# sydney-machine-learning/parallel-tempering-neural-net

Measured on AMD Instinct MI355X. Metric: MCMC samples/sec (all replicas) + swap-accept rate; Sunspot 64-replica FNN, higher is better.
Workload: dtype f32

## Files before the change

### parallel-tempering-neural-net_amd/csrc/ptnn.hip

```cpp
#include "ptnn_shapes.hpp"
namespace ptnn {
#include "ptnn_dev_swap.hpp"
}
#include "ptnn_host.hpp"

#include <algorithm>
#include <atomic>
#include <cmath>
#include <cstdarg>
#include <cstdio>
#include <cstdlib>
#include <cstring>
#include <memory>
#include <unordered_map>
#include <mutex>
#include <string>
#include <thread>
#include <vector>
#include <sched.h>

using namespace ptnn;

thread_local std::string ptnn::g_err;

// ... 152 lines not shown
void ladder_adapt_release(ptnn_handle* h) {
    for (void* p : {(void*)h->d_lad_hist, (void*)h->d_lad_s, (void*)h->d_lad_acc})
        if (p) (void)hipFree(p);
    h->d_lad_hist = nullptr; h->d_lad_s = nullptr; h->d_lad_acc = nullptr;
    h->have_adapt = false; h->adapt = ptnn_ladder_adapt_spec{};
    h->lad_T0.clear(); h->lad_s0.clear();
}

}

int ptnn::ladder_adapt_alloc(ptnn_handle* h, const ptnn_ladder_adapt_spec& spec) {
    ladder_adapt_release(h);
    const size_t R = h->cfg.n_replicas_global;
    HIP_TRY(hipMalloc(&h->d_lad_hist, (size_t)(spec.rounds + 1) * R * sizeof(float)));
    HIP_TRY(hipMalloc(&h->d_lad_s, 2 * (R - 1) * sizeof(double)));
    HIP_TRY(hipMalloc(&h->d_lad_acc, (size_t)h->max_rounds * (R - 1) * sizeof(float)));
    h->adapt = spec; h->have_adapt = true;
    return 0;
}

namespace {

int ladder_adapt_reset(ptnn_handle* h) {
    const size_t R = h->cfg.n_replicas_global;
    HIP_TRY(hipMemsetAsync(h->d_lad_hist, 0xff, (size_t)(h->adapt.rounds + 1) * R * sizeof(float), h->stream));
    HIP_TRY(hipMemsetAsync(h->d_lad_acc, 0xff, (size_t)h->max_rounds * (R - 1) * sizeof(float), h->stream));
    HIP_TRY(hipMemcpyAsync(h->d_lad_hist, h->lad_T0.data(), R * sizeof(float), hipMemcpyHostToDevice, h->stream));
    HIP_TRY(hipMemcpyAsync(h->d_temps_global, h->lad_T0.data(), R * sizeof(float), hipMemcpyHostToDevice, h->stream));
    HIP_TRY(hipMemcpyAsync(h->d_lad_s, h->lad_s0.data(), (R - 1) * sizeof(double), hipMemcpyHostToDevice, h->stream));
    HIP_TRY(hipStreamSynchronize(h->stream));
    return 0;
}

int launch_segment(ptnn_handle* h, int begin, int end, bool swap_inside = false, bool round_follows = false) {
    if (end <= begin) return 0;
    HIP_TRY(hipSetDevice(h->cfg.device_id));
    SegParams p = h->seg_params();
    if (round_follows && h->comm.kind == COMM_RCCL) { p.seg_progress = h->h_progress + 1; p.seg_ordinal = h->rounds_done + 1; }
    PersistParams pp{};
    pp.end = end; pp.swap_inside = swap_inside ? 1 : 0; pp.task = h->cfg.task; pp.si = h->cfg.swap_interval;
    pp.round0 = h->rounds_done; pp.flip0 = h->flip; pp.lflip0 = h->lflip;
    const int grid = h->plan.grid(h->cfg.n_replicas_local);
    pp.nblocks = grid; pp.barrier = h->d_barrier;
    for (int b = 0; b < 2; ++b) {
        pp.state[b] = h->d_state[b]; pp.gd[b] = h->d_gd_w[b]; pp.gd_valid[b] = h->d_gd_valid[b];
        pp.label[b] = h->d_label[b]; pp.slot_of[b] = h->d_slot_of[b];
    }
    fill_swap_params(h, false, pp.sp);
    if (swap_inside) {
        if (grid > h->barrier_slots) {
            if (h->d_barrier) HIP_TRY(hipFree(h->d_barrier));
            h->d_barrier = nullptr;
            HIP_TRY(hipMalloc(&h->d_barrier, (size_t)grid * sizeof(unsigned)));
            h->barrier_slots = grid;
            pp.barrier = h->d_barrier;
        }
        HIP_TRY(hipMemsetAsync(h->d_barrier, 0, (size_t)grid * sizeof(unsigned), h->stream));
    }
    const bool timed = h->timing_stride > 0 && (h->launch_count++ % h->timing_stride) == 0;
    std::pair<hipEvent_t, hipEvent_t>* ev = nullptr;
    if (timed) {
        if (h->timing_used == h->timing.size()) {
            if (h->timing.size() >= 4096) {
                if (int rc = wait_stream(h)) return rc;
                collect_timing(h);
            } else {
                hipEvent_t a, b;
                HIP_TRY(hipEventCreate(&a));
                HIP_TRY(hipEventCreate(&b));
                h->timing.emplace_back(a, b);
            }
        }
        ev = &h->timing[h->timing_used++];
        HIP_TRY(hipEventRecord(ev->first, h->stream));
    }
    hipLaunchKernelGGL(plan_function(h->shape, h->plan), dim3(grid), dim3(h->plan.threads), h->plan.seg_lds, h->stream, p, pp, begin);
    h->epoch_base += (unsigned)(end - begin) + 1u + (swap_inside ? (unsigned)((end - begin) / h->cfg.swap_interval + 2) : 0u);
    HIP_TRY(hipGetLastError());
    if (ev) HIP_TRY(hipEventRecord(ev->second, h->stream));
    return 0;
}

int launch_swap(ptnn_handle* h, bool phantom, int mode, bool want_src) {
    HIP_TRY(hipSetDevice(h->cfg.device_id));
    SwapParams sp{};
    fill_swap_params(h, phantom, sp);
    sp.src_out = want_src ? h->d_src : nullptr;
    sp.progress = (mode >= 0 && (mode & 2)) ? h->h_progress : nullptr;
    if (mode == -1) {
        hipLaunchKernelGGL(xchg_pack_kernel, dim3(sp.Rl), dim3(64), 0, h->stream, sp);
// ... 263 lines not shown
        if (explicit_tree && want) break;
    }
    if (explicit_tree)
        return fail(-3, "tree schedule: %d replicas x %d work-groups of %d threads cannot all be resident on %d CUs (or need more than "
                        "160 KiB of LDS)", Rl, want ? want : 3, threads, h.num_cus);
    return 0;
}

int plan_persistent(const ptnn_handle& h, LaunchPlan& plan) {
    const ptnn_config& c = h.cfg;
    const char* e = std::getenv("PTNN_PERSISTENT");
    if ((e && e[0] == '0') || c.shared_device) return 0;
    const bool forced = e && e[0] == '1';
    const int R = c.n_replicas_global;
    const bool whole = c.swap_rule == 0 && !c.label_swap && plan.xswap > 0 && c.n_replicas_local == R;
    const bool tree_inside = plan.kind == SEG_TREE && whole && R <= TREE_PERSIST_MAX_R;
    const bool packm_inside = plan.kind == SEG_PACKM && whole && (size_t)(3 * R + 1) <= (size_t)pack_slots(plan.pk_nred) * pack_slot_floats(h.PS);
    const bool own_rounds = tree_inside || packm_inside;
    if (plan.grid(1) > 1 && !own_rounds && !forced) return 0;
    if (c.swap_interval < 8 && !own_rounds && !forced) return 0;
    if (plan.kind == SEG_SPEC || (plan.kind == SEG_TREE && !tree_inside) || (plan.kind == SEG_PACKM && !packm_inside)) return 0;
    if (plan.kind == SEG_PACK && !(h.shape->loops & 2)) return 0;
    if (plan.kind == SEG_COOP && !(h.shape->loops & 1)) return 0;
    const size_t swap_lds = (size_t)(3 * R + 1) * sizeof(float);
    if (swap_lds > plan.seg_lds) {
        if (swap_lds > LDS_CEILING) return 0;
        plan.seg_lds = swap_lds;
    }
    const void* fn = reinterpret_cast<const void*>(plan_function(h.shape, plan));
    if (int rc = raise_lds_limit(fn, plan.seg_lds)) return rc;
    int per_cu = 0;
    HIP_TRY(hipOccupancyMaxActiveBlocksPerMultiprocessor(&per_cu, fn, plan.threads, plan.seg_lds));
    plan.persistent = (long long)plan.grid(c.n_replicas_local) <= (long long)per_cu * h.num_cus;
    return 0;
}

int plan_launch(const ptnn_handle& h, int Nall, int Npad, LaunchPlan& plan) {
    const ptnn_config& c = h.cfg;
    plan = LaunchPlan{};
    if (c.n_hidden > WAVE) {
        if (int rc = plan_wide(h, plan)) return rc;
    } else {
        plan.model_lds = lds_floats(Nall, h.IPY, h.PS, c.n_hidden, h.FWS) * sizeof(float);
        if (plan.model_lds > LDS_MAX)
            return fail(-3, "replica working set needs %zu B of LDS (> 160 KiB): data %d rows x %d floats, P = %d", plan.model_lds, Nall,
                        h.IPY, h.P);
        int sched = c.schedule;
        if (sched == PTNN_SCHED_AUTO) sched = (c.task == PTNN_TASK_REG || c.use_langevin) ? PTNN_SCHED_SPECULATIVE : PTNN_SCHED_COOPERATIVE;
        if (sched != PTNN_SCHED_COOPERATIVE && sched != PTNN_SCHED_SPECULATIVE && sched != PTNN_SCHED_PACKED && sched != PTNN_SCHED_TREE)
            return fail(-1, "unknown schedule %d", sched);
        if (sched == PTNN_SCHED_TREE && (c.task != PTNN_TASK_CLS || c.use_langevin))
            return fail(-3, "the prefetching tree schedule is built for random-walk classification runs");
        plan.pk_nred = (c.n_hidden <= 8) ? 3 : 4;
        if (int rc = plan_packed(h, Nall, sched, plan)) return rc;
        if (plan.kind != SEG_COOP) sched = PTNN_SCHED_PACKED;
        const int nw = c.waves_per_replica;
        if (nw != 0 && nw != 1 && nw != 2 && nw != 4 && nw != 8) return fail(-1, "waves_per_replica must be 0 (auto), 1, 2, 4 or 8");
        int pow2 = 1;
        while (pow2 < (Nall + 63) / 64) pow2 <<= 1;
        plan.model_threads = std::min(pow2, 8) * 64;
        if (sched == PTNN_SCHED_SPECULATIVE) {
            if (int rc = plan_speculative(h, Nall, plan)) return rc;
            if (plan.kind == SEG_COOP) sched = PTNN_SCHED_COOPERATIVE;
        }
        if (sched == PTNN_SCHED_COOPERATIVE) plan_cooperative(h, Nall, Npad, plan);
        const bool auto_tree = sched == PTNN_SCHED_COOPERATIVE && c.schedule == PTNN_SCHED_AUTO && c.task == PTNN_TASK_CLS &&
// ... 185 lines not shown
    int ndev = 0;
    HIP_TRY(hipGetDeviceCount(&ndev));
    if (cfg->device_id < 0 || cfg->device_id >= ndev) return fail(-2, "device %d not present (%d devices)", cfg->device_id, ndev);
    HIP_TRY(hipSetDevice(cfg->device_id));
    hipDeviceProp_t prop;
    HIP_TRY(hipGetDeviceProperties(&prop, cfg->device_id));
    if (std::strncmp(prop.gcnArchName, "gfx950", 6) != 0)
        return fail(-2, "device %d is %s; libptnn is built for gfx950 only", cfg->device_id, prop.gcnArchName);

    if (cfg->trace_capacity < 0 || (cfg->trace_capacity > 0 && cfg->trace_capacity < 2))
        return fail(-1, "trace_capacity must be 0 (= n_samples) or >= 2");
    ptnn_handle* h = new ptnn_handle();
    if (int rc = create_buffers(h, cfg, sh, prop)) {
        const std::string why = g_err;
        ptnn_destroy(h);
        g_err = why;
        return rc;
    }
    *out = h;
    return 0;
}

int ptnn_destroy(ptnn_handle* h) {
    if (!h) return 0;
    (void)hipSetDevice(h->cfg.device_id);
    if (h->stream && !h->comm.failed) (void)wait_stream(h);
    h->comm.release();
    if (h->comm.failed && h->stream) {
        const double t0 = comm_clock();
        while (hipStreamQuery(h->stream) == hipErrorNotReady && comm_clock() - t0 < 5.0) std::this_thread::sleep_for(std::chrono::milliseconds(1));
        if (hipStreamQuery(h->stream) == hipErrorNotReady) return fail(-7, "the stream of a failed communicator did not drain: handle leaked");
    }
    void* ptrs[] = {h->d_data, h->d_state[0], h->d_state[1], h->d_rec_w, h->d_gd_w[0], h->d_gd_w[1], h->d_gd_valid[0], h->d_gd_valid[1], h->d_st_f, h->d_st_i, h->d_temps,
                    h->d_L_handoff, h->d_L_final, h->d_L_raw, h->d_prior_post, h->d_temps_global, h->d_pos_w, h->d_scal, h->d_src, h->d_label[0], h->d_label[1], h->d_slot_of[0], h->d_slot_of[1], h->d_src_log, h->d_counters, h->d_error, h->d_xslots, h->d_xw, h->d_xverdict, h->d_xswap, h->d_stamps, h->d_wide_scratch, h->d_xt, h->d_xs, h->d_barrier};
    for (void* p : ptrs)
        if (p) (void)hipFree(p);
    if (h->h_src) (void)hipHostFree(h->h_src);
    if (h->h_progress) (void)hipHostFree(h->h_progress);
    if (h->h_stage) (void)hipHostFree(h->h_stage);
    if (h->d_stage) (void)hipFree(h->d_stage);
    if (h->d_xchg) (void)hipFree(h->d_xchg);
    ladder_adapt_release(h);
    for (auto& ev : h->timing) { (void)hipEventDestroy(ev.first); (void)hipEventDestroy(ev.second); }
    if (h->copy_stream) { (void)hipStreamSynchronize(h->copy_stream); (void)hipStreamDestroy(h->copy_stream); }
    for (auto& ev : h->img_events) (void)hipEventDestroy(ev);
    if (h->h_img_pos) (void)hipHostFree(h->h_img_pos);
    if (h->h_img_rows) (void)hipHostFree(h->h_img_rows);
    if (h->stream) (void)hipStreamDestroy(h->stream);
    delete h;
    return 0;
}

int ptnn_set_data(ptnn_handle* h, const float* train, int ntr, const float* test, int nte, int ncols) {
    if (!h || !train || !test) return fail(-1, "null argument");
    if (ncols < h->cfg.n_in + 1) return fail(-1, "data needs at least n_in + 1 = %d columns, got %d", h->cfg.n_in + 1, ncols);
    if (ntr < 1 || nte < 1) return fail(-1, "empty data set");
    HIP_TRY(hipSetDevice(h->cfg.device_id));
    DataImages img;
    if (int rc = pack_data(*h, train, ntr, test, nte, ncols, img)) return rc;
    LaunchPlan plan;
    if (int rc = plan_launch(*h, ntr + nte, img.Npad, plan)) return rc;
    return apply_plan(h, img, plan);
}

int ptnn_set_state(ptnn_handle* h, const float* w0, const float* temperatures) {
    if (!h || !w0 || !temperatures) return fail(-1, "null argument");
    if (!h->have_data) return fail(-1, "call ptnn_set_data before ptnn_set_state");
// ... 802 lines not shown
    ms[0] = ticks(0) / (double)khz / (double)reps;
    ms[1] = ticks(2) / (double)khz / (double)reps / 2.0;
    ms[2] = (double)out[5];
    return 0;
}

int ptnn_tape(ptnn_handle* h, int replica, int step, float* noise, float* scal) {
    if (!h || !noise || !scal) return fail(-1, "null argument");
    const size_t off = h->plan.wide() ? (size_t)h->PS : (size_t)h->P;
    std::vector<float> buf(off + 3);
    if (int rc = run_model(h, 2, nullptr, nullptr, 1, buf.data(), buf.size(), replica, step)) return rc;
    std::memcpy(noise, buf.data(), h->P * sizeof(float));
    std::memcpy(scal, buf.data() + off, 3 * sizeof(float));
    return 0;
}

int ptnn_describe(ptnn_handle* h, char* buf, int nbytes) {
    if (!h || !buf || nbytes < 1) return fail(-1, "bad argument");
    if (!h->have_data) return fail(-1, "ptnn_set_data has not been called (the schedule depends on the data set)");
    const LaunchPlan& pl = h->plan;
    const void* fn = reinterpret_cast<const void*>(plan_function(h->shape, pl));
    HIP_TRY(hipSetDevice(h->cfg.device_id));
    char width[16] = "";
    if ((pl.kind == SEG_PACK || pl.kind == SEG_PACKM) && pl.pack_hc > 0) std::snprintf(width, sizeof width, ",%d", pl.pack_hc);
    int per_cu = 0;
    HIP_TRY(hipOccupancyMaxActiveBlocksPerMultiprocessor(&per_cu, fn, pl.threads, pl.seg_lds));
    hipFuncAttributes fa{};
    HIP_TRY(hipFuncGetAttributes(&fa, fn));
    const int slots = pl.kind == SEG_COOP ? 1
                    : pl.kind == SEG_SPEC ? pl.groups * (pl.threads / WAVE)
                    : pl.kind == SEG_TREE ? tree_depth(pl.groups)
                    : pl.wide() ? (pl.groups > 1 && h->cfg.use_langevin ? 8 : pl.groups)
                    : pack_slots(pl.pk_nred) * pl.groups;
    const int n = std::snprintf(buf, (size_t)nbytes,
                                "{\"kernel\": \"ptnn::%s<%d,%d,%d%s>\", \"schedule\": \"%s\", \"grid_blocks\": %d, \"block_threads\": %d, "
                                "\"lds_bytes\": %zu, \"groups_per_replica\": %d, \"slots_per_round\": %d, \"num_cus\": %d, "
                                "\"blocks_per_cu\": %d, \"vgprs\": %d, \"scratch_bytes\": %zu, \"forward_mfma\": %d, \"exchange\": \"%s\", \"lds_resident_state\": %d, \"compact_traces\": %d, \"launches\": \"%s\"}",
                                g_seg[pl.kind].name, h->cfg.task, h->cfg.n_in, h->cfg.n_out, width,
                                pl.wide() && pl.groups > 1 ? "speculative-wide" : g_seg[pl.kind].label,
                                pl.grid(h->cfg.n_replicas_local), pl.threads, pl.seg_lds, pl.groups, slots, h->num_cus, per_cu, fa.numRegs, (size_t)fa.localSizeBytes,
                                pl.fw_mfma ? pl.fw_mfma : ((pl.wide() && h->cfg.n_hidden % 32 == 0) ? 1 : 0),
                                h->comm.kind == COMM_NONE ? "none" : (h->cfg.label_swap ? "labels" : (resolved_xchg_mode(h) == PTNN_XCHG_GATHER ? "gather" : "boundary")),
                                pl.kind == SEG_WIDE_RES ? 1 : 0, pl.compact ? 1 : 0,
                                (pl.persistent && h->comm.kind == COMM_NONE) ? "one per ptnn_run (swap rounds inside)" : "one per swap interval");
    if (n < 0 || n >= nbytes) return fail(-1, "buffer of %d bytes is too small for the description", nbytes);
    return n;
}

int ptnn_kernel_time(ptnn_handle* h, int reset, int64_t* launches, double* total_ms) {
    if (!h) return fail(-1, "null handle");
    HIP_TRY(hipSetDevice(h->cfg.device_id));
    if (int rc = wait_stream(h)) return rc;
    collect_timing(h);
    if (launches) *launches = h->timed_launches;
    if (total_ms) *total_ms = h->timed_ms;
    if (reset) { h->timed_launches = 0; h->timed_ms = 0.0; }
    return 0;
}

int ptnn_debug_stamps(ptnn_handle* h, uint64_t* out16) {
    if (!h || !out16) return fail(-1, "null argument");
    HIP_TRY(hipSetDevice(h->cfg.device_id));
    if (int rc = wait_stream(h)) return rc;
    HIP_TRY(hipMemcpy(out16, h->d_stamps, 160 * sizeof(unsigned long long), hipMemcpyDeviceToHost));
    HIP_TRY(hipMemset(h->d_stamps, 0, 160 * sizeof(unsigned long long)));
    const unsigned long long big = ~0ull;
    HIP_TRY(hipMemcpy(h->d_stamps + 12, &big, sizeof big, hipMemcpyHostToDevice));
    return 0;
}

}
```

### parallel-tempering-neural-net_amd/csrc/ptnn_dev_kernels.hpp

```cpp

template <int TASK, int I, int O>
__global__ void __launch_bounds__(MAX_THREADS) model_kernel(const SegParams p, const int mode, const float* __restrict__ w_in,
                             const float* __restrict__ tau_sq, float* __restrict__ out, int a0, int a1) {
    extern __shared__ __attribute__((aligned(16))) float smem[];
    const int b = blockIdx.x, tid = threadIdx.x, nthr = blockDim.x;
    const int Nall = p.Ntr + p.Nte;
    const Lds l = carve(smem, Nall, p.IPY, p.PS, p.H, p.FWS);
    if (mode == 2) {
        tape_step(p, a0, a1, l.noise, l.scal);
        __syncthreads();
        for (int j = tid; j < p.P; j += nthr) out[j] = l.noise[j];
        if (tid < 3) out[p.P + tid] = l.scal[tid];
        return;
    }
    {
        const float4* src = reinterpret_cast<const float4*>(p.data);
        float4* dst = reinterpret_cast<float4*>(l.xy);
        for (int e = tid; e < ((Nall + 2) * p.IPY) >> 2; e += nthr) dst[e] = src[e];
    }
    for (int j = tid; j < p.P; j += nthr) l.w_cur[j] = w_in[(size_t)(mode == 4 ? 0 : b) * p.P + j];
    __syncthreads();
    if (mode == 4) {
        granule_t* const ga = reinterpret_cast<granule_t*>(out + 16);
        granule_t* const gb = ga + 8;
// ... 67 lines not shown
    const float ss = block_sumsq(l.w_cur, p.P, l.red);
    const float pr = prior_value<TASK>(p, ss, eta);
    float ll_te = s.a_te;
    if (TASK == TASK_REG) ll_te = -0.5f * (float)p.Nte * (LOG_2PI + eta) - 0.5f * s.a_te * expf_fast(-eta);
    if (tid == 0) {
        float* o = out + (size_t)b * 8;
        o[0] = ll; o[1] = r1; o[2] = r2; o[3] = a_tr; o[4] = a_te; o[5] = pr; o[6] = ll_te; o[7] = 0.f;
    }
}

__device__ __forceinline__ bool grid_barrier(unsigned* slots, int nblocks, unsigned phase, int* error_flag) {
    __syncthreads();
    int bad = 0;
    if (threadIdx.x < WAVE) {
        if (threadIdx.x == 0) {
            __builtin_amdgcn_fence(__ATOMIC_RELEASE, "agent");
            __hip_atomic_store(slots + blockIdx.x, phase, __ATOMIC_RELAXED, __HIP_MEMORY_SCOPE_AGENT);
        }
        unsigned spins = 0;
        for (;;) {
            bool here = true;
            for (int j = threadIdx.x; j < nblocks; j += WAVE)
                here = here && (__hip_atomic_load(slots + j, __ATOMIC_RELAXED, __HIP_MEMORY_SCOPE_AGENT) >= phase);
            if (__all(here)) break;
            __builtin_amdgcn_s_sleep(4);
            if (++spins > SPIN_LIMIT || __hip_atomic_load(error_flag, __ATOMIC_RELAXED, __HIP_MEMORY_SCOPE_AGENT) != 0) { bad = 1; break; }
        }
    }
    bad = __syncthreads_or(bad);
    __builtin_amdgcn_fence(__ATOMIC_ACQUIRE, "agent");
    return bad == 0;
}

template <bool LOOP, class Body>
__device__ __forceinline__ void persistent_loop(const SegParams& p0, const int step_begin, Body body) {
    extern __shared__ __attribute__((aligned(16))) float smem[];
    if constexpr (!LOOP) {
        const SegParams& p = p0;
        persist_cptr pp = persist_args();
        SegDyn dyn;
        const int flip = pp->flip0;
        dyn.pp = pp;
        dyn.w_state = pp->state[flip]; dyn.gd_w = pp->gd[flip]; dyn.gd_valid = pp->gd_valid[flip];
        dyn.epoch_base = p.epoch_base;
        body(p, dyn, step_begin, pp->end - step_begin);
        if (p.seg_progress && blockIdx.x == 0 && threadIdx.x == 0)
            __hip_atomic_store(p.seg_progress, p.seg_ordinal, __ATOMIC_RELAXED, __HIP_MEMORY_SCOPE_SYSTEM);
        return;
    }
    int flip, lflip, round, cur = step_begin;
    unsigned phase = 0, epoch_add = 0;
    {
        persist_cptr pp = persist_args();
        flip = pp->flip0; lflip = pp->lflip0; round = pp->round0;
    }
    for (;;) {
        persist_cptr pp = persist_args();
        const int end = pp->end, si = pp->si;
        if (cur >= end) break;
        int seg_end;
        if (pp->task == TASK_REG) { const int c1 = cur > 1 ? cur : 1; seg_end = ((c1 + si - 1) / si) * si; }
        else seg_end = ((cur + si) / si) * si - 1;
        const bool handoff = seg_end < end;
        const int stop = handoff ? seg_end + 1 : end;
        const bool swap_inside = pp->swap_inside != 0;
#if defined(__HIP_DEVICE_COMPILE__)
        const SegParams p = *seg_args();
#else
        const SegParams p = p0;
#endif
        {
            SegDyn dyn;
            dyn.pp = pp;
            dyn.w_state = pp->state[flip]; dyn.gd_w = pp->gd[flip]; dyn.gd_valid = pp->gd_valid[flip];
            dyn.epoch_base = p.epoch_base + epoch_add;
            body(p, dyn, cur, stop - cur);
        }
        epoch_add += (unsigned)(stop - cur) + 1u;
        cur = stop;
        if (!handoff || !swap_inside) break;
        pp = persist_args();
        if (!grid_barrier(pp->barrier, pp->nblocks, ++phase, p.error_flag)) { if (threadIdx.x == 0) atomicAdd(p.error_flag, 1); return; }
        if (xcd_block(p.G) % p.G == 0) {
#if defined(__HIP_DEVICE_COMPILE__)
            SwapParams sp = pp->sp;
#else
            SwapParams sp{};
#endif
            sp.cur = pp->state[flip]; sp.next = pp->state[flip ^ 1];
            sp.gd_cur = pp->gd[flip]; sp.gd_next = pp->gd[flip ^ 1];
            sp.gd_valid_cur = pp->gd_valid[flip]; sp.gd_valid_next = pp->gd_valid[flip ^ 1];
            sp.label_cur = pp->label[lflip]; sp.slot_cur = pp->slot_of[lflip];
            sp.label_next = pp->label[lflip ^ 1]; sp.slot_next = pp->slot_of[lflip ^ 1];
            sp.canonical = (p.switch_step >= 0 && cur - 1 >= p.switch_step) ? 1 : 0;
            if (sp.lad_hist) sp.temps_global = sp.lad_hist + (size_t)min(round, sp.lad_A) * sp.R;
            swap_block(sp, round, 3, xcd_block(p.G) / p.G, smem);
        }
        if (pp->sp.label_mode) lflip ^= 1; else flip ^= 1;
        round += 1;
        if (p.G > 1 && !grid_barrier(pp->barrier, pp->nblocks, ++phase, p.error_flag)) { if (threadIdx.x == 0) atomicAdd(p.error_flag, 1); return; }
        if (p.G == 1) __syncthreads();
    }
    if (p0.seg_progress && blockIdx.x == 0 && threadIdx.x == 0)
        __hip_atomic_store(p0.seg_progress, p0.seg_ordinal, __ATOMIC_RELAXED, __HIP_MEMORY_SCOPE_SYSTEM);
}

template <int TASK, int I, int O> constexpr bool coop_has_loop() { return O <= 3; }
template <int TASK, int I, int O> constexpr bool pack_has_loop() { return TASK == TASK_REG && I <= 8; }

template <int TASK, int I, int O>
__global__ void __launch_bounds__(MAX_THREADS) segment_kernel(const SegParams p, const PersistParams pp, const int step_begin) {
    persistent_loop<coop_has_loop<TASK, I, O>()>(p, step_begin, [](const SegParams& q, const SegDyn& d, int b, int n) { segment_body<TASK, I, O>(q, d, b, n); });
}
template <int TASK, int I, int O>
__global__ void __launch_bounds__(MAX_THREADS) segment_spec_kernel(const SegParams p, const PersistParams pp, const int step_begin) {
    persistent_loop<false>(p, step_begin, [](const SegParams& q, const SegDyn& d, int b, int n) { segment_spec_body<TASK, I, O>(q, d, b, n); });
}
template <int TASK, int I, int O>
__global__ void __launch_bounds__(PK_WAVES * WAVE) segment_pack_kernel(const SegParams p, const PersistParams pp, const int step_begin) {
    persistent_loop<pack_has_loop<TASK, I, O>()>(p, step_begin, [](const SegParams& q, const SegDyn& d, int b, int n) {
        if (q.pk_nred == 4) segment_pack_body<TASK, I, O, 4>(q, d, b, n);
        else segment_pack_body<TASK, I, O, 3>(q, d, b, n);
    });
}
template <int TASK, int I, int O, int HC>
__global__ void __launch_bounds__(PK_WAVES * WAVE) segment_pack_kernel(const SegParams p, const PersistParams pp, const int step_begin) {
    static_assert(HC > 0 && HC <= 16, "a packed net has at most 16 hidden units");
    persistent_loop<pack_has_loop<TASK, I, O>()>(p, step_begin, [](const SegParams& q, const SegDyn& d, int b, int n) {
        segment_pack_body<TASK, I, O, pack_nred(HC), false, HC>(q, d, b, n);
    });
}
template <int TASK, int I, int O>
__global__ void __launch_bounds__(PK_WAVES * WAVE) segment_packm_kernel(const SegParams p, const PersistParams pp, const int step_begin) {
    persistent_loop<false>(p, step_begin, [](const SegParams& q, const SegDyn& d, int b, int n) {
        if (q.pk_nred == 4) segment_pack_body<TASK, I, O, 4, true>(q, d, b, n);
        else segment_pack_body<TASK, I, O, 3, true>(q, d, b, n);
    });
}
template <int TASK, int I, int O, int HC>
__global__ void __launch_bounds__(PK_WAVES * WAVE) segment_packm_kernel(const SegParams p, const PersistParams pp, const int step_begin) {
    static_assert(HC > 0 && HC <= 16, "a packed net has at most 16 hidden units");
    persistent_loop<false>(p, step_begin, [](const SegParams& q, const SegDyn& d, int b, int n) {
        segment_pack_body<TASK, I, O, pack_nred(HC), true, HC>(q, d, b, n);
    });
}
template <int TASK, int I, int O>
__global__ void __launch_bounds__(MAX_THREADS) segment_tree_kernel(const SegParams p, const PersistParams pp, const int step_begin) {
    persistent_loop<false>(p, step_begin, [](const SegParams& q, const SegDyn& d, int b, int n) { segment_tree_body<TASK, I, O>(q, d, b, n); });
}
#pragma clang fp contract(fast)
template <int TASK, int I, int O>
__global__ void __launch_bounds__(MAX_THREADS) segment_wide_kernel(const SegParams p, const PersistParams pp, const int step_begin) {
    persistent_loop<true>(p, step_begin, [](const SegParams& q, const SegDyn& d, int b, int n) { segment_wide_body<TASK, I, O, false>(q, d, b, n); });
}
template <int TASK, int I, int O>
__global__ void __launch_bounds__(MAX_THREADS) segment_wide_res_kernel(const SegParams p, const PersistParams pp, const int step_begin) {
    persistent_loop<true>(p, step_begin, [](const SegParams& q, const SegDyn& d, int b, int n) { segment_wide_body<TASK, I, O, true>(q, d, b, n); });
}
#pragma clang fp contract(off)
```

### parallel-tempering-neural-net_amd/csrc/ptnn_dev_spec.hpp

```cpp

enum { SL_ACCEPT = 0, SL_LIKPROP, SL_PRIORPROP, SL_ETAPRO, SL_RM_TR, SL_RM_TE, SL_AC_TR, SL_AC_TE, SL_LG, SL_ADAPT, SL_LOGALPHA, SL_D2, SL_COUNT = 16 };
constexpr int MAX_SLOTS = 64;
constexpr unsigned SPIN_LIMIT = 1u << 22;

__host__ __device__ inline size_t spec_wave_floats(int PS, int H, int FWS) { return 3 * (size_t)PS + fw_floats(H, FWS) + 8; }
__host__ __device__ inline size_t spec_lds_floats(int Nall, int IPY, int PS, int H, int FWS, int NW, int G) {
    return (size_t)(Nall + 2) * IPY + 3 * (size_t)PS + MAX_WAVES * 8 + 32 + (size_t)NW * G * SL_COUNT + (size_t)NW * spec_wave_floats(PS, H, FWS);
}

typedef unsigned long long granule_t;
__device__ __forceinline__ void granule_store(granule_t* g, unsigned epoch, float v) {
    __hip_atomic_store(g, ((granule_t)epoch << 32) | (granule_t)__builtin_bit_cast(unsigned, v), __ATOMIC_RELAXED,
                       __HIP_MEMORY_SCOPE_AGENT);
}
__device__ __forceinline__ bool granule_wait(const granule_t* g, unsigned epoch, float& v) {
    for (unsigned spins = 0; spins < SPIN_LIMIT; ++spins) {
        const granule_t x = __hip_atomic_load(g, __ATOMIC_RELAXED, __HIP_MEMORY_SCOPE_AGENT);
        if ((unsigned)(x >> 32) == epoch) { v = __builtin_bit_cast(float, (unsigned)x); return true; }
        __builtin_amdgcn_s_sleep(2);
    }
    return false;
}
__device__ __forceinline__ int xcc_id() {
    int x;
// ... 50 lines not shown
    float* next;
    const float* gd_cur;
    float* gd_next;
    const int* gd_valid_cur;
    int* gd_valid_next;
    int* src_out;
    long long* counters;
    int* src_log;
    int log_capacity;
    int rule, canonical;
    const float* L_raw;
    const float* prior_post;
    const float* temps_global;
    float* st_f;
    float* xchg;
    int XS;
    int L_stride;
    int label_mode;
    const int* label_cur;
    const int* slot_cur;
    int* label_next;
    int* slot_next;
    float* temps_local;
    int* progress;
    float* lad_hist;
    double* lad_s;
    float* lad_acc;
    float* lad_out;
    int lad_A, lad_acc_cap;
    double lad_kappa0, lad_t0;
};
__host__ __device__ inline int xchg_row_floats(int PS) { return (2 * PS + 4 + 3) & ~3; }

__device__ __forceinline__ int cascade_lds(const SwapParams& sp, int round, float* sL, float* sU, int* sSrc, bool have_L = false) {
    const int R = sp.R;
    for (int k = threadIdx.x; k < R; k += blockDim.x) {
        if (!have_L) sL[k] = sp.L[(size_t)(sp.label_mode ? sp.slot_cur[k] : k) * sp.L_stride];
        if (k < R - 1) {
            uint32_t x[4];
            philox4x32_10((uint32_t)k, (uint32_t)round, 0u, STREAM_SWAP, sp.seed_lo, sp.seed_hi, x);
            sU[k] = (sp.rule == 1) ? u23(x[0]) : logf_fast(2.0f * u23(x[0]));
        }
    }
    __syncthreads();
    if (sp.rule == 1) {
        for (int k = threadIdx.x; k < R; k += blockDim.x) sSrc[k] = k;
        if (threadIdx.x == 0) sSrc[R] = 0;
        __syncthreads();
        for (int k = (round & 1) + 2 * threadIdx.x; k < R - 1; k += 2 * blockDim.x) {
            const int s0 = sp.label_mode ? sp.slot_cur[k] : k, s1 = sp.label_mode ? sp.slot_cur[k + 1] : k + 1;
            const float d = (1.0f / sp.temps_global[k] - 1.0f / sp.temps_global[k + 1]) *
                            (sp.L_raw[(size_t)s1 * sp.L_stride] - sp.L_raw[(size_t)s0 * sp.L_stride]);
            const float pr = (d != d) ? 1.0f : fminf(1.0f, expf_fast(fminf(d, 80.0f)));
            if (sU[k] < pr) { sSrc[k] = k + 1; sSrc[k + 1] = k; atomicAdd(&sSrc[R], 1); }
        }
        __syncthreads();
        return sSrc[R];
    }
    if (threadIdx.x < WAVE) {
        const int lane = threadIdx.x;
        int c = 0, nsw = 0;
        float Lc = sL[0];
        for (int k0 = 0; k0 < R - 1; k0 += WAVE) {
            const int k = k0 + lane;
            const bool valid = k < R - 1;
            const float Ln = valid ? sL[k + 1] : 0.0f;
            const float tk = valid ? sU[k] : 0.0f;
            unsigned long long todo = __ballot(valid);
            unsigned long long swapped = 0ull;
            while (todo) {
                float d = Ln - Lc;
                d = (d < 709.0f) ? d : 709.0f;
                const unsigned long long fail = __ballot(!(tk < d)) & todo;
                if (!fail) { swapped |= todo; break; }
                const int j = __ffsll((long long)fail) - 1;
                swapped |= todo & ((1ull << j) - 1ull);
                if (lane == j) sSrc[k] = c;
                c = k0 + j + 1;
                Lc = __shfl(Ln, j);
                todo &= (j == 63) ? 0ull : ~((2ull << j) - 1ull);
            }
            if (valid && ((swapped >> lane) & 1ull)) sSrc[k] = k + 1;
            nsw += __popcll(swapped);
        }
        if (lane == 0) { sSrc[R - 1] = c; sSrc[R] = nsw; }
    }
    __syncthreads();
    return sSrc[R];
}

struct PersistParams {
    int end;
    int swap_inside;
    int task, si;
    int round0;
    int flip0, lflip0;
    int nblocks;
    unsigned* barrier;
    float* state[2];
    float* gd[2];
    int* gd_valid[2];
    int* label[2];
    int* slot_of[2];
    SwapParams sp;
};

__device__ __forceinline__ persist_cptr persist_args() {
    constexpr size_t off = (sizeof(SegParams) + alignof(PersistParams) - 1) & ~(alignof(PersistParams) - 1);
    unsigned long long a = (unsigned long long)(uintptr_t)__builtin_amdgcn_kernarg_segment_ptr() + off;
    asm volatile("" : "+s"(a));
    return (persist_cptr)(uintptr_t)a;
}

typedef __attribute__((address_space(4))) const SegParams* seg_cptr;
__device__ __forceinline__ seg_cptr seg_args() {
    unsigned long long a = (unsigned long long)(uintptr_t)__builtin_amdgcn_kernarg_segment_ptr();
    asm volatile("" : "+s"(a));
    return (seg_cptr)(uintptr_t)a;
}

__host__ __device__ inline size_t swap_xchg_granules(int R, int row) { return (size_t)((R + 7) & ~7) + (size_t)R * row + (size_t)R * (row + 8); }

template <int TASK, int I, int O>
__device__ __forceinline__ void segment_spec_body(const SegParams& p, const SegDyn& dyn, const int step_begin, const int n_steps) {
    extern __shared__ __attribute__((aligned(16))) float smem[];
    PTNN_DIAG(spec_entry);
    const int G = p.G;
    const int lb = xcd_block(G);
    const int r = lb / G, grp = lb - r * G;
    const int gid = p.first_global + r;
    const int tid = threadIdx.x, nthr = blockDim.x;
    const int wave = tid >> 6, lane = tid & 63, NW = nthr >> 6;
    const int K = NW * G;
    const int sidx = grp * NW + wave;
    const int Nall = p.Ntr + p.Nte;
    const int P = p.P, PS = p.PS, H = p.H;
    float* q = smem;
    float* xy = q; q += (Nall + 2) * p.IPY;
// ... 308 lines not shown
```

### parallel-tempering-neural-net_amd/csrc/ptnn_host.hpp

```cpp
#pragma once
#include "ptnn_comm.hpp"
#include "ptnn_dims.hpp"
#include "../../include/ptnn.h"

#include <cstdint>
#include <string>
#include <utility>
#include <vector>

#pragma GCC visibility push(hidden)

namespace ptnn {

struct Shape;
struct SegParams;

extern thread_local std::string g_err;

int fail(int code, const char* fmt, ...);

#define HIP_TRY(expr)                                                                                      \
    do {                                                                                                   \
        hipError_t e_ = (expr);                                                                            \
        if (e_ != hipSuccess) {                                                                            \
            (void)hipGetLastError();    \
            return fail(-2, "%s failed: %s (%s:%d)", #expr, hipGetErrorString(e_), __FILE__, __LINE__);    \
        }                                                                                                  \
    } while (0)

constexpr size_t LDS_MAX = 160 * 1024;
constexpr size_t LDS_CEILING = 152 * 1024;

enum SegKind { SEG_COOP, SEG_SPEC, SEG_PACK, SEG_PACKM, SEG_TREE, SEG_WIDE, SEG_WIDE_RES, SEG_KINDS };

struct LaunchPlan {
    SegKind kind = SEG_COOP;
    int threads = 64, model_threads = 64;
    size_t seg_lds = 0, model_lds = 0;
    int groups = 1;
    int pk_nred = 3;
    int pack_hc = 0;
    int fw_mfma = 0;
    bool xy_global = false;
    bool tree_ahead = false;
    bool compact = false;
    int blocks_per_cu = 0;
    bool persistent = false;
    size_t xslots = 0, xw = 0, xverdict = 0, xswap = 0, wide_scratch = 0;
    bool wide() const { return kind == SEG_WIDE || kind == SEG_WIDE_RES; }
    int grid(int replicas) const;
};

}

struct ptnn_handle {
    ptnn_config cfg{};
    const ptnn::Shape* shape = nullptr;
    hipStream_t stream = nullptr;
    int P = 0, PS = 0, PW = 0, IPY = 0, FWS = 0, Ntr = 0, Nte = 0;
    ptnn::LaunchPlan plan;
    unsigned* d_barrier = nullptr;
    int barrier_slots = 0;
    float* d_wide_scratch = nullptr;
    float* d_xt = nullptr;
    uint16_t* d_xs = nullptr;
    int Npad = 0;
    unsigned epoch_base = 0;
    int num_cus = 0;
    unsigned long long *d_xslots = nullptr, *d_xw = nullptr, *d_xverdict = nullptr, *d_xswap = nullptr;
    int* d_error = nullptr;
    float *h_stage = nullptr, *d_stage = nullptr;
    int* h_progress = nullptr;
    bool failed = false;
    std::string failure;
    unsigned long long* d_stamps = nullptr;
    bool have_data = false, have_state = false, finalized = false;
    int cap = 0;
    int drained = 0;
    int first_row = 0;
    int cur = 0;
    int rounds_done = 0;
    int max_rounds = 0;
    int flip = 0;
    float* d_data = nullptr;
    float* d_state[2] = {nullptr, nullptr};
    float *d_rec_w = nullptr, *d_st_f = nullptr, *d_temps = nullptr;
    float* d_gd_w[2] = {nullptr, nullptr};
    int* d_gd_valid[2] = {nullptr, nullptr};
    int* d_st_i = nullptr;
    float *d_L_handoff = nullptr, *d_L_final = nullptr;
    float *d_L_raw = nullptr, *d_prior_post = nullptr, *d_temps_global = nullptr;
    bool have_ladder = false;
    bool have_adapt = false;
    ptnn_ladder_adapt_spec adapt{};
    float* d_lad_hist = nullptr;
// ... 39 lines not shown
```

Measured before the change: 17.02 million.

## Pipeline in-kernel replica swaps through a ring buffer instead of a grid barrier

```diff
diff --git a/parallel-tempering-neural-net_amd/csrc/ptnn.hip b/parallel-tempering-neural-net_amd/csrc/ptnn.hip
--- a/parallel-tempering-neural-net_amd/csrc/ptnn.hip
+++ b/parallel-tempering-neural-net_amd/csrc/ptnn.hip
@@ -208,6 +208,10 @@
     return 0;
 }
 
+bool swap_pipelined(const ptnn_handle* h) {
+    return h->plan.persistent && h->plan.swap_pipeline && h->comm.kind == COMM_NONE && !h->have_adapt;
+}
+
 int launch_segment(ptnn_handle* h, int begin, int end, bool swap_inside = false, bool round_follows = false) {
     if (end <= begin) return 0;
     HIP_TRY(hipSetDevice(h->cfg.device_id));
@@ -232,6 +236,26 @@
             pp.barrier = h->d_barrier;
         }
         HIP_TRY(hipMemsetAsync(h->d_barrier, 0, (size_t)grid * sizeof(unsigned), h->stream));
+    }
+    pp.delay_replica = -1;
+    if (swap_inside && swap_pipelined(h)) {
+        const int R = h->cfg.n_replicas_global;
+        const int row = swap_ring_row_floats(h->PS);
+        if (R > h->swap_ring_replicas) {
+            for (void* q : {(void*)h->d_swap_ring, (void*)h->d_swap_tags})
+                if (q) HIP_TRY(hipFree(q));
+            h->d_swap_ring = nullptr; h->d_swap_tags = nullptr; h->swap_ring_replicas = 0;
+            HIP_TRY(hipMalloc(&h->d_swap_ring, (size_t)SWAP_RING_DEPTH * R * (row + 1) * sizeof(float)));
+            HIP_TRY(hipMalloc(&h->d_swap_tags, (size_t)2 * R * sizeof(unsigned)));
+            h->swap_ring_replicas = R;
+        }
+        HIP_TRY(hipMemsetAsync(h->d_swap_tags, 0, (size_t)2 * R * sizeof(unsigned), h->stream));
+        pp.pipeline = 1; pp.ring_row = row; pp.ring = h->d_swap_ring; pp.ring_L = h->d_swap_ring + (size_t)SWAP_RING_DEPTH * R * row; pp.ready = h->d_swap_tags; pp.taken = h->d_swap_tags + R;
+        if (h->plan.delay_replica >= 0 && h->plan.delay_us > 0) {
+            int khz = 0;
+            HIP_TRY(hipDeviceGetAttribute(&khz, hipDeviceAttributeWallClockRate, h->cfg.device_id));
+            if (khz > 0) { pp.delay_replica = h->plan.delay_replica; pp.delay_ticks = (unsigned)((long long)h->plan.delay_us * khz / 1000); }
+        }
     }
     const bool timed = h->timing_stride > 0 && (h->launch_count++ % h->timing_stride) == 0;
     std::pair<hipEvent_t, hipEvent_t>* ev = nullptr;
@@ -561,6 +585,14 @@
     int per_cu = 0;
     HIP_TRY(hipOccupancyMaxActiveBlocksPerMultiprocessor(&per_cu, fn, plan.threads, plan.seg_lds));
     plan.persistent = (long long)plan.grid(c.n_replicas_local) <= (long long)per_cu * h.num_cus;
+    const char* pe = std::getenv("PTNN_SWAP_PIPELINE");
+    plan.swap_pipeline = plan.persistent && !(pe && pe[0] == '0') && plan.kind == SEG_PACK && plan.grid(1) == 1 && c.swap_rule == 0 &&
+                         !c.label_swap && c.n_replicas_local == R;
+    if (const char* de = std::getenv("PTNN_SWAP_DELAY")) {
+        constexpr int SWAP_DELAY_MAX_US = 5000;
+        int r = -1, t = 0;
+        if (std::sscanf(de, "%d:%d", &r, &t) == 2 && r >= 0 && r < R && t > 0) { plan.delay_replica = r; plan.delay_us = std::min(t, SWAP_DELAY_MAX_US); }
+    }
     return 0;
 }
 
@@ -812,7 +844,7 @@
         if (hipStreamQuery(h->stream) == hipErrorNotReady) return fail(-7, "the stream of a failed communicator did not drain: handle leaked");
     }
     void* ptrs[] = {h->d_data, h->d_state[0], h->d_state[1], h->d_rec_w, h->d_gd_w[0], h->d_gd_w[1], h->d_gd_valid[0], h->d_gd_valid[1], h->d_st_f, h->d_st_i, h->d_temps,
-                    h->d_L_handoff, h->d_L_final, h->d_L_raw, h->d_prior_post, h->d_temps_global, h->d_pos_w, h->d_scal, h->d_src, h->d_label[0], h->d_label[1], h->d_slot_of[0], h->d_slot_of[1], h->d_src_log, h->d_counters, h->d_error, h->d_xslots, h->d_xw, h->d_xverdict, h->d_xswap, h->d_stamps, h->d_wide_scratch, h->d_xt, h->d_xs, h->d_barrier};
+                    h->d_L_handoff, h->d_L_final, h->d_L_raw, h->d_prior_post, h->d_temps_global, h->d_pos_w, h->d_scal, h->d_src, h->d_label[0], h->d_label[1], h->d_slot_of[0], h->d_slot_of[1], h->d_src_log, h->d_counters, h->d_error, h->d_xslots, h->d_xw, h->d_xverdict, h->d_xswap, h->d_stamps, h->d_wide_scratch, h->d_xt, h->d_xs, h->d_barrier, h->d_swap_ring, h->d_swap_tags};
     for (void* p : ptrs)
         if (p) (void)hipFree(p);
     if (h->h_src) (void)hipHostFree(h->h_src);
@@ -1681,17 +1713,23 @@
                     : pl.kind == SEG_TREE ? tree_depth(pl.groups)
                     : pl.wide() ? (pl.groups > 1 && h->cfg.use_langevin ? 8 : pl.groups)
                     : pack_slots(pl.pk_nred) * pl.groups;
+    const bool inside = pl.persistent && h->comm.kind == COMM_NONE;
+    const bool pipelined = swap_pipelined(h);
+    const char* const swap_rounds = !inside ? "between launches" : pipelined ? "pipelined (ring 4)"
+                                    : (pl.kind == SEG_TREE || pl.kind == SEG_PACKM) ? "in-kernel exchange" : "grid barrier";
+    static_assert(SWAP_RING_DEPTH == 4, "describe() spells the ring depth out");
     const int n = std::snprintf(buf, (size_t)nbytes,
                                 "{\"kernel\": \"ptnn::%s<%d,%d,%d%s>\", \"schedule\": \"%s\", \"grid_blocks\": %d, \"block_threads\": %d, "
                                 "\"lds_bytes\": %zu, \"groups_per_replica\": %d, \"slots_per_round\": %d, \"num_cus\": %d, "
-                                "\"blocks_per_cu\": %d, \"vgprs\": %d, \"scratch_bytes\": %zu, \"forward_mfma\": %d, \"exchange\": \"%s\", \"lds_resident_state\": %d, \"compact_traces\": %d, \"launches\": \"%s\"}",
+                                "\"blocks_per_cu\": %d, \"vgprs\": %d, \"scratch_bytes\": %zu, \"forward_mfma\": %d, \"exchange\": \"%s\", \"lds_resident_state\": %d, \"compact_traces\": %d, \"launches\": \"%s\", \"swap_rounds\": \"%s\", \"swap_ring_depth\": %d}",
                                 g_seg[pl.kind].name, h->cfg.task, h->cfg.n_in, h->cfg.n_out, width,
                                 pl.wide() && pl.groups > 1 ? "speculative-wide" : g_seg[pl.kind].label,
                                 pl.grid(h->cfg.n_replicas_local), pl.threads, pl.seg_lds, pl.groups, slots, h->num_cus, per_cu, fa.numRegs, (size_t)fa.localSizeBytes,
                                 pl.fw_mfma ? pl.fw_mfma : ((pl.wide() && h->cfg.n_hidden % 32 == 0) ? 1 : 0),
                                 h->comm.kind == COMM_NONE ? "none" : (h->cfg.label_swap ? "labels" : (resolved_xchg_mode(h) == PTNN_XCHG_GATHER ? "gather" : "boundary")),
                                 pl.kind == SEG_WIDE_RES ? 1 : 0, pl.compact ? 1 : 0,
-                                (pl.persistent && h->comm.kind == COMM_NONE) ? "one per ptnn_run (swap rounds inside)" : "one per swap interval");
+                                (pl.persistent && h->comm.kind == COMM_NONE) ? "one per ptnn_run (swap rounds inside)" : "one per swap interval",
+                                swap_rounds, pipelined ? (int)SWAP_RING_DEPTH : 0);
     if (n < 0 || n >= nbytes) return fail(-1, "buffer of %d bytes is too small for the description", nbytes);
     return n;
 }
diff --git a/parallel-tempering-neural-net_amd/csrc/ptnn_dev_kernels.hpp b/parallel-tempering-neural-net_amd/csrc/ptnn_dev_kernels.hpp
--- a/parallel-tempering-neural-net_amd/csrc/ptnn_dev_kernels.hpp
+++ b/parallel-tempering-neural-net_amd/csrc/ptnn_dev_kernels.hpp
@@ -123,7 +123,100 @@
     return bad == 0;
 }
 
-template <bool LOOP, class Body>
+__device__ __forceinline__ int poll_reached(const unsigned* words, int n, unsigned want, int* error_flag) {
+    int bad = 0;
+    if (threadIdx.x < WAVE) {
+        unsigned spins = 0;
+        for (;;) {
+            bool here = true;
+            for (int j = threadIdx.x; j < n; j += WAVE)
+                here = here && (__hip_atomic_load(words + j, __ATOMIC_RELAXED, __HIP_MEMORY_SCOPE_AGENT) >= want);
+            if (__all(here)) break;
+            __builtin_amdgcn_s_sleep(4);
+            if (++spins > SPIN_LIMIT || __hip_atomic_load(error_flag, __ATOMIC_RELAXED, __HIP_MEMORY_SCOPE_AGENT) != 0) { bad = 1; break; }
+        }
+    }
+    return bad;
+}
+
+__device__ __forceinline__ bool swap_handoff(persist_cptr pp, const int flip, const int round, const unsigned n, int* error_flag, float* smem) {
+    const int R = pp->sp.R, PS = pp->sp.PS, ROW = pp->ring_row;
+    const int k = blockIdx.x;
+    float* const slot = pp->ring + (size_t)(n % SWAP_RING_DEPTH) * R * ROW;
+    float* const slot_L = pp->ring_L + (size_t)(n % SWAP_RING_DEPTH) * R;
+    __syncthreads();
+    if (pp->delay_replica == k) {
+        const unsigned long long t0 = wall_clock64();
+        for (unsigned s = 0; s < SPIN_LIMIT && wall_clock64() - t0 < (unsigned long long)pp->delay_ticks; ++s) __builtin_amdgcn_s_sleep(8);
+    }
+    if (n >= SWAP_RING_DEPTH) {
+        if (__syncthreads_or(poll_reached(pp->taken, R, n - SWAP_RING_DEPTH + 1u, error_flag))) return false;
+    }
+    {
+        const float4* const w = reinterpret_cast<const float4*>(pp->state[flip] + (size_t)k * PS);
+        const float4* const g = reinterpret_cast<const float4*>(pp->gd[flip] + (size_t)k * PS);
+        float* const row = slot + (size_t)k * ROW;
+        for (int j = threadIdx.x; j < PS / 4; j += blockDim.x) {
+            reinterpret_cast<float4*>(row)[j] = w[j];
+            reinterpret_cast<float4*>(row + PS)[j] = g[j];
+        }
+        if (threadIdx.x == 0) {
+            reinterpret_cast<int*>(row)[2 * PS] = pp->gd_valid[flip][k];
+            slot_L[k] = pp->sp.L[pp->sp.first_global + k];
+        }
+    }
+    asm volatile("s_waitcnt vmcnt(0)" ::: "memory");
+    __syncthreads();
+    if (threadIdx.x == 0) {
+        __builtin_amdgcn_fence(__ATOMIC_RELEASE, "agent");
+        asm volatile("s_waitcnt vmcnt(0)" ::: "memory");
+        __hip_atomic_store(pp->ready + k, n + 1u, __ATOMIC_RELAXED, __HIP_MEMORY_SCOPE_AGENT);
+    }
+    const int Rp = min(k + 2, R);
+    const int bad = __syncthreads_or(poll_reached(pp->ready, Rp, n + 1u, error_flag));
+    __builtin_amdgcn_fence(__ATOMIC_ACQUIRE, "agent");
+    if (bad) return false;
+    float* const sL = smem;
+    float* const sU = smem + R;
+    int* const sSrc = reinterpret_cast<int*>(smem + 2 * R);
+    for (int j = threadIdx.x; j < Rp; j += blockDim.x) sL[j] = slot_L[j];
+#if defined(__HIP_DEVICE_COMPILE__)
+    const SwapParams sp = pp->sp;
+#else
+    const SwapParams sp{};
+#endif
+    const int nsw = cascade_lds_prefix(sp, Rp, round, sL, sU, sSrc, true);
+    if (k == R - 1) {
+        if (sp.src_out) for (int j = threadIdx.x; j < R; j += blockDim.x) sp.src_out[j] = sSrc[j];
+        if (sp.src_log && round < sp.log_capacity)
+            for (int j = threadIdx.x; j < R; j += blockDim.x) sp.src_log[(size_t)round * R + j] = sSrc[j];
+        if (threadIdx.x == 0) {
+            sp.counters[0] += nsw;
+            sp.counters[1] += R - 1;
+            if (sp.progress) __hip_atomic_store(sp.progress, round + 1, __ATOMIC_RELAXED, __HIP_MEMORY_SCOPE_SYSTEM);
+        }
+    }
+    {
+        const float* const from = slot + (size_t)sSrc[k] * ROW;
+        float4* const w = reinterpret_cast<float4*>(pp->state[flip ^ 1] + (size_t)k * PS);
+        float4* const g = reinterpret_cast<float4*>(pp->gd[flip ^ 1] + (size_t)k * PS);
+        for (int j = threadIdx.x; j < PS / 4; j += blockDim.x) {
+            w[j] = reinterpret_cast<const float4*>(from)[j];
+            g[j] = reinterpret_cast<const float4*>(from + PS)[j];
+        }
+        if (threadIdx.x == 0) pp->gd_valid[flip ^ 1][k] = reinterpret_cast<const int*>(from)[2 * PS];
+    }
+    asm volatile("s_waitcnt vmcnt(0)" ::: "memory");
+    __syncthreads();
+    if (threadIdx.x == 0) {
+        __builtin_amdgcn_fence(__ATOMIC_RELEASE, "agent");
+        asm volatile("s_waitcnt vmcnt(0)" ::: "memory");
+        __hip_atomic_store(pp->taken + k, n + 1u, __ATOMIC_RELAXED, __HIP_MEMORY_SCOPE_AGENT);
+    }
+    return true;
+}
+
+template <bool LOOP, bool PIPE = false, class Body>
 __device__ __forceinline__ void persistent_loop(const SegParams& p0, const int step_begin, Body body) {
     extern __shared__ __attribute__((aligned(16))) float smem[];
     if constexpr (!LOOP) {
@@ -171,6 +264,14 @@
         cur = stop;
         if (!handoff || !swap_inside) break;
         pp = persist_args();
+        if constexpr (PIPE) {
+            if (pp->pipeline) {
+                if (!swap_handoff(pp, flip, round, phase++, p.error_flag, smem)) { if (threadIdx.x == 0) atomicAdd(p.error_flag, 1); return; }
+                flip ^= 1;
+                round += 1;
+                continue;
+            }
+        }
         if (!grid_barrier(pp->barrier, pp->nblocks, ++phase, p.error_flag)) { if (threadIdx.x == 0) atomicAdd(p.error_flag, 1); return; }
         if (xcd_block(p.G) % p.G == 0) {
 #if defined(__HIP_DEVICE_COMPILE__)
@@ -209,7 +310,7 @@
 }
 template <int TASK, int I, int O>
 __global__ void __launch_bounds__(PK_WAVES * WAVE) segment_pack_kernel(const SegParams p, const PersistParams pp, const int step_begin) {
-    persistent_loop<pack_has_loop<TASK, I, O>()>(p, step_begin, [](const SegParams& q, const SegDyn& d, int b, int n) {
+    persistent_loop<pack_has_loop<TASK, I, O>(), true>(p, step_begin, [](const SegParams& q, const SegDyn& d, int b, int n) {
         if (q.pk_nred == 4) segment_pack_body<TASK, I, O, 4>(q, d, b, n);
         else segment_pack_body<TASK, I, O, 3>(q, d, b, n);
     });
@@ -217,7 +318,7 @@
 template <int TASK, int I, int O, int HC>
 __global__ void __launch_bounds__(PK_WAVES * WAVE) segment_pack_kernel(const SegParams p, const PersistParams pp, const int step_begin) {
     static_assert(HC > 0 && HC <= 16, "a packed net has at most 16 hidden units");
-    persistent_loop<pack_has_loop<TASK, I, O>()>(p, step_begin, [](const SegParams& q, const SegDyn& d, int b, int n) {
+    persistent_loop<pack_has_loop<TASK, I, O>(), true>(p, step_begin, [](const SegParams& q, const SegDyn& d, int b, int n) {
         segment_pack_body<TASK, I, O, pack_nred(HC), false, HC>(q, d, b, n);
     });
 }
diff --git a/parallel-tempering-neural-net_amd/csrc/ptnn_dev_spec.hpp b/parallel-tempering-neural-net_amd/csrc/ptnn_dev_spec.hpp
--- a/parallel-tempering-neural-net_amd/csrc/ptnn_dev_spec.hpp
+++ b/parallel-tempering-neural-net_amd/csrc/ptnn_dev_spec.hpp
@@ -106,8 +106,7 @@
 };
 __host__ __device__ inline int xchg_row_floats(int PS) { return (2 * PS + 4 + 3) & ~3; }
 
-__device__ __forceinline__ int cascade_lds(const SwapParams& sp, int round, float* sL, float* sU, int* sSrc, bool have_L = false) {
-    const int R = sp.R;
+__device__ __forceinline__ int cascade_lds_prefix(const SwapParams& sp, const int R, int round, float* sL, float* sU, int* sSrc, bool have_L) {
     for (int k = threadIdx.x; k < R; k += blockDim.x) {
         if (!have_L) sL[k] = sp.L[(size_t)(sp.label_mode ? sp.slot_cur[k] : k) * sp.L_stride];
         if (k < R - 1) {
@@ -162,6 +161,9 @@
     __syncthreads();
     return sSrc[R];
 }
+__device__ __forceinline__ int cascade_lds(const SwapParams& sp, int round, float* sL, float* sU, int* sSrc, bool have_L = false) {
+    return cascade_lds_prefix(sp, sp.R, round, sL, sU, sSrc, have_L);
+}
 
 struct PersistParams {
     int end;
@@ -177,7 +179,17 @@
     int* label[2];
     int* slot_of[2];
     SwapParams sp;
+    int pipeline;
+    int ring_row;
+    float* ring;
+    float* ring_L;
+    unsigned* ready;
+    unsigned* taken;
+    int delay_replica;
+    unsigned delay_ticks;
 };
+constexpr unsigned SWAP_RING_DEPTH = 4;
+__host__ __device__ inline int swap_ring_row_floats(int PS) { return 2 * PS + 4; }
 
 __device__ __forceinline__ persist_cptr persist_args() {
     constexpr size_t off = (sizeof(SegParams) + alignof(PersistParams) - 1) & ~(alignof(PersistParams) - 1);
diff --git a/parallel-tempering-neural-net_amd/csrc/ptnn_host.hpp b/parallel-tempering-neural-net_amd/csrc/ptnn_host.hpp
--- a/parallel-tempering-neural-net_amd/csrc/ptnn_host.hpp
+++ b/parallel-tempering-neural-net_amd/csrc/ptnn_host.hpp
@@ -46,6 +46,9 @@
     bool compact = false;
     int blocks_per_cu = 0;
     bool persistent = false;
+    bool swap_pipeline = false;
+    int delay_replica = -1;
+    int delay_us = 0;
     size_t xslots = 0, xw = 0, xverdict = 0, xswap = 0, wide_scratch = 0;
     bool wide() const { return kind == SEG_WIDE || kind == SEG_WIDE_RES; }
     int grid(int replicas) const;
@@ -61,6 +64,9 @@
     ptnn::LaunchPlan plan;
     unsigned* d_barrier = nullptr;
     int barrier_slots = 0;
+    float* d_swap_ring = nullptr;
+    unsigned* d_swap_tags = nullptr;
+    int swap_ring_replicas = 0;
     float* d_wide_scratch = nullptr;
     float* d_xt = nullptr;
     uint16_t* d_xs = nullptr;
```

Result: faster. 19.15 million (median of 6 runs) (+12.5%).
